# azmyrajab/polars_ols

Hardware: AMD Instinct MI355X
Metric: group_regressions_per_sec (higher is better)
Workload: dtype f32

## Files before the change

### polars_ols_amd/csrc/k4x_inverse.hip

```cpp
#include "k4_rolling.hpp"

namespace pols {

constexpr int KX_MAX = 128;

template <typename T>
struct XCtx {
    const K4Args &a;
    int64_t s;
    int first_chunk;
    int K, LD, NS, tid;
    double *P, *xs, *v, *bv, *beta, *red;
    const T *mycol;
    __device__ XCtx(const K4Args &a_, int64_t s_, int fc, double *lds) : a(a_), s(s_), first_chunk(fc) {
        K = a.k; LD = K | 1; NS = K * K + K; tid = threadIdx.x;
        P = lds; xs = P + (size_t)K * LD; v = xs + KX_MAX + 2; bv = v + KX_MAX; beta = bv + KX_MAX; red = beta + KX_MAX;
        mycol = tid < K ? static_cast<const T *>(a.xtab ? a.xtab[tid] : a.x[tid]) : static_cast<const T *>(a.y);
    }
    static __host__ __device__ size_t lds_doubles(int K) { return (size_t)K * (K | 1) + 4 * KX_MAX + 2 + 16; }

    __device__ __forceinline__ bool valid(int64_t i) const { return a.valid ? a.valid[s + i] != 0 : true; }
    __device__ __forceinline__ int64_t cnt(int64_t i) const { return a.cnt ? (int64_t)a.cnt[s + i] : i + 1; }
    __device__ __forceinline__ int64_t vidx(int64_t r) const { return a.vidx ? (int64_t)a.vidx[s + r] : r; }

    __device__ __forceinline__ void load_row(int64_t i) const {
        __syncthreads();
        if (tid <= K) xs[tid] = (double)mycol[s + i];
        __syncthreads();
    }
    __device__ double block_sum(double x) const {
        const double w = wave_sum_row3(x);
        __syncthreads();
        if ((tid & 63) == 63) red[tid >> 6] = w;
        __syncthreads();
        return red[0] + red[1] + red[2] + red[3];
    }
    __device__ void zero() const {
        for (int q = tid; q < K * LD; q += 256) P[q] = 0.0;
        if (tid < K) bv[tid] = 0.0;
        __syncthreads();
    }
    __device__ void gram_axpy(const double *src, double sign) const {
        for (int q = tid; q < K * K; q += 256) { const int i = q / K, c = q - i * K; P[i * LD + c] += sign * src[q]; }
        if (tid < K) bv[tid] += sign * src[K * K + tid];
        __syncthreads();
    }
    __device__ void gram_add_row(int64_t i, double sign) const {
        load_row(i);
        for (int q = tid; q < K * K; q += 256) { const int r = q / K, c = q - r * K; P[r * LD + c] += sign * (xs[r] * xs[c]); }
        if (tid < K) bv[tid] += sign * (xs[tid] * xs[K]);
        __syncthreads();
    }
    __device__ void gram_prefix(int64_t i, double sign, int nacc) const {
        if (i < 0) return;
        const int64_t c = i / a.chunk_len;
        gram_axpy(a.totals + (size_t)(first_chunk + c) * nacc, sign);
        for (int64_t j = c * a.chunk_len; j <= i; ++j)
            if (valid(j)) gram_add_row(j, sign);
    }
    __device__ void invert(double alpha) const {
        if (tid < K) P[tid * LD + tid] += alpha;
        __syncthreads();
        for (int j = 0; j < K; ++j) {
            const double p = 1.0 / P[j * LD + j];
            if (tid < K) v[tid] = P[tid * LD + j];
            __syncthreads();
            for (int q = tid; q < K * K; q += 256) {
                const int i = q / K, c = q - i * K;
                double val;
                if (i == j && c == j) val = -p;
                else if (i == j) val = v[c] * p;
                else if (c == j) val = v[i] * p;
                else val = P[i * LD + c] - v[i] * v[c] * p;
                P[i * LD + c] = val;
            }
            __syncthreads();
        }
        for (int q = tid; q < K * K; q += 256) { const int i = q / K, c = q - i * K; P[i * LD + c] = -P[i * LD + c]; }
        __syncthreads();
    }
    __device__ void matvec(const double *x, double *out) const {
        if (tid < K) {
            double acc = 0.0;
            const double *row = P + tid * LD;
            for (int c = 0; c < K; ++c) acc += row[c] * x[c];
            out[tid] = acc;
        }
        __syncthreads();
    }
    __device__ void rank1(double coef) const {
        for (int q = tid; q < K * K; q += 256) { const int i = q / K, c = q - i * K; P[i * LD + c] += coef * (v[i] * v[c]); }
        __syncthreads();
    }
    __device__ void sm_update(double sign) const {
        matvec(xs, v);
        const double xv = block_sum(tid < K ? xs[tid] * v[tid] : 0.0);
        rank1(-sign / (1.0 + sign * xv));
        if (tid < K) bv[tid] += sign * (xs[tid] * xs[K]);
        __syncthreads();
    }
    __device__ void solve_beta() const { matvec(bv, beta); }
    __device__ void store(int64_t i, bool have, T *coef, T *pred) const {
        const int64_t row = s + i;
        const double qnan = __longlong_as_double(0x7ff8000000000000LL);
        if (coef && tid < K) coef[row * K + tid] = (T)(have ? beta[tid] : qnan);
        if (pred) {
            load_row(i);
            const double p = block_sum(tid < K ? xs[tid] * (have ? beta[tid] : qnan) : 0.0);
            if (tid == 0) pred[row] = (T)p;
        }
    }
};

template <typename T, bool RLS>
__global__ void __launch_bounds__(256) kx_totals_kernel(const K4Args a) {
    extern __shared__ double lds[];
    const int64_t c = blockIdx.x;
    const K4Chunk ch = a.chunks[c];
    const K4Group G = a.groups[ch.group];
    XCtx<T> cx(a, G.start, G.first_chunk, lds);
    const int K = cx.K, nacc = cx.NS + (RLS ? 1 : 0);
    cx.zero();
    double decay = 1.0;
    for (int64_t i = ch.t0 - G.start; i < ch.t1 - G.start; ++i)
        if (cx.valid(i)) {
            if (RLS) {
                for (int q = cx.tid; q < K * cx.LD; q += 256) cx.P[q] *= a.ff;
                if (cx.tid < K) cx.bv[cx.tid] *= a.ff;
                decay *= a.ff;
                __syncthreads();
            }
            cx.gram_add_row(i, 1.0);
        }
    double *out = a.totals + (size_t)c * nacc;
    for (int q = cx.tid; q < K * K; q += 256) { const int i = q / K, cc = q - i * K; out[q] = cx.P[i * cx.LD + cc]; }
    if (cx.tid < K) out[K * K + cx.tid] = cx.bv[cx.tid];
    if (RLS && cx.tid == 0) out[cx.NS] = decay;
}

template <typename T>
__global__ void __launch_bounds__(256) kx_rolling_walk_kernel(const K4Args a) {
    extern __shared__ double lds[];
    const int64_t c = blockIdx.x;
    const K4Chunk ch = a.chunks[c];
    const K4Group G = a.groups[ch.group];
    XCtx<T> cx(a, G.start, G.first_chunk, lds);
    const int K = cx.K, nacc = cx.NS;
    const int64_t rel0 = ch.t0 - G.start, rel1 = ch.t1 - G.start;
    const int64_t w = a.window, mpv = G.mpv;
    const bool drop = a.drop_mode != 0;
    T *coef = static_cast<T *>(a.coef);
    T *pred = static_cast<T *>(a.pred);
    const double qnan = __longlong_as_double(0x7ff8000000000000LL);

    if (G.all_nan) {
        for (int64_t i = rel0; i < rel1; ++i) {
            if (coef && cx.tid < K) coef[(G.start + i) * K + cx.tid] = (T)qnan;
            if (pred && cx.tid == 0) pred[G.start + i] = (T)qnan;
        }
        return;
    }
    const int64_t j_min = drop ? 0 : max(mpv - w, (int64_t)0);
    const int64_t c0 = drop ? cx.cnt(mpv - 1) : 0;
    const bool longwarm = drop && c0 > w;
    auto old_of = [&](int64_t i) -> int64_t {
        if (!drop) return i - w;
        const int64_t R = cx.cnt(i) - 1;
        const int64_t r = (longwarm && R - c0 < w) ? R - c0 : R - w;
        return r < 0 ? -1 : cx.vidx(r);
    };
    auto gate = [&](int64_t i) -> bool {
        const int64_t i_start = i >= w ? i - w : 0;
        return cx.cnt(i) - cx.cnt(i_start) >= G.gate_n;
    };
    auto gram_state_at = [&](int64_t i) {
        cx.zero();
        cx.gram_prefix(i, 1.0, nacc);
        const int64_t o = (i >= 0) ? old_of(i) : -1;
        if (o >= j_min && i >= mpv) {
            cx.gram_prefix(o, -1.0, nacc);
            cx.gram_prefix(j_min - 1, 1.0, nacc);
        }
        if (longwarm && i >= mpv && cx.cnt(i) - 1 - c0 >= w) {
            cx.gram_prefix(cx.vidx(c0 - 1), 1.0, nacc);
            cx.gram_prefix(cx.vidx(w - 1), -1.0, nacc);
        }
    };

    bool inverted = false, have = false;
    int64_t prev_old = (rel0 > 0 && rel0 - 1 >= mpv) ? old_of(rel0 - 1) : -1;
    if (rel0 >= mpv && rel0 > 0) {
        int64_t ip = rel0 - 1;
        if (!(drop || ip == mpv - 1 || gate(ip))) {
            for (ip = rel0 - 2; ip >= mpv - 1; --ip)
                if (ip == mpv - 1 || gate(ip)) break;
        }
        gram_state_at(ip);
        cx.invert(a.alpha);
        cx.solve_beta();
        have = true;
        if (ip != rel0 - 1) {
            gram_state_at(rel0 - 1);
            cx.invert(a.alpha);
        }
        inverted = true;
    } else {
        gram_state_at(rel0 - 1);
    }
    for (int64_t i = rel0; i < rel1; ++i) {
        const bool vld = cx.valid(i);
        if (vld) {
            if (inverted) { cx.load_row(i); cx.sm_update(1.0); }
            else cx.gram_add_row(i, 1.0);
        }
        if (i >= mpv && (vld || !drop)) {
            const int64_t no = old_of(i);
            bool sub = false;
            if (drop) sub = (no != prev_old && no >= 0);
            else sub = (no >= j_min && no >= 0 && cx.valid(no));
            if (sub) { cx.load_row(no); cx.sm_update(-1.0); }
            prev_old = no;
        }
        if (i >= mpv - 1) {
            const bool do_solve = (i == mpv - 1) || (drop ? vld : gate(i));
            if (do_solve) {
                if (!inverted) { cx.invert(a.alpha); inverted = true; }
                cx.solve_beta();
                have = true;
            }
        }
        cx.store(i, have, coef, pred);
    }
}

template <typename T>
__global__ void __launch_bounds__(256) kx_rls_walk_kernel(const K4Args a) {
    extern __shared__ double lds[];
    const int64_t c = blockIdx.x;
    const K4Chunk ch = a.chunks[c];
    const K4Group G = a.groups[ch.group];
    XCtx<T> cx(a, G.start, G.first_chunk, lds);
    const int K = cx.K, nacc = cx.NS + 1;
    const int64_t rel0 = ch.t0 - G.start, rel1 = ch.t1 - G.start;
    T *coef = static_cast<T *>(a.coef);
    T *pred = static_cast<T *>(a.pred);
    cx.zero();
    cx.gram_axpy(a.totals + (size_t)c * nacc, 1.0);
    cx.invert(0.0);
    cx.solve_beta();
    const double ff = a.ff;
    for (int64_t i = rel0; i < rel1; ++i) {
        if (cx.valid(i)) {
            cx.load_row(i);
            cx.matvec(cx.xs, cx.v);
            const double xv = cx.block_sum(cx.tid < K ? cx.xs[cx.tid] * cx.v[cx.tid] : 0.0);
            const double xb = cx.block_sum(cx.tid < K ? cx.xs[cx.tid] * cx.beta[cx.tid] : 0.0);
            const double r = 1.0 + xv / ff;
            const double err = cx.xs[K] - xb;
            if (cx.tid < K) cx.beta[cx.tid] += cx.v[cx.tid] / (r * ff) * err;
            const double coef_vv = -1.0 / (r * ff);
            for (int q = cx.tid; q < K * K; q += 256) {
                const int ii = q / K, cc = q - ii * K;
                cx.P[ii * cx.LD + cc] = (cx.P[ii * cx.LD + cc] + coef_vv * (cx.v[ii] * cx.v[cc])) / ff;
            }
            __syncthreads();
        }
        cx.store(i, true, coef, pred);
    }
}

template <typename T>
static int kx_launch_t(pols_ctx *ctx, const K4Args &a, bool rls) {
    const size_t lds = sizeof(double) * XCtx<T>::lds_doubles(a.k);
    const int ns = a.k * a.k + a.k;
    static OncePerDevice attr_once;
    if (attr_once.needed(ctx->device)) {
        const void *fns[4] = {reinterpret_cast<const void *>(&kx_totals_kernel<T, false>), reinterpret_cast<const void *>(&kx_totals_kernel<T, true>),
                              reinterpret_cast<const void *>(&kx_rolling_walk_kernel<T>), reinterpret_cast<const void *>(&kx_rls_walk_kernel<T>)};
        for (const void *f : fns) POLS_HIP(hipFuncSetAttribute(f, hipFuncAttributeMaxDynamicSharedMemorySize, 144 * 1024));
        attr_once.done(ctx->device);
    }
    timing_begin(ctx);
    if (rls) {
        hipLaunchKernelGGL((kx_totals_kernel<T, true>), dim3((unsigned)a.n_chunks), dim3(256), lds, ctx->stream, a);
        chunk_scan_launch(ctx, a, ns, 2);
        hipLaunchKernelGGL((kx_rls_walk_kernel<T>), dim3((unsigned)a.n_chunks), dim3(256), lds, ctx->stream, a);
    } else {
        hipLaunchKernelGGL((kx_totals_kernel<T, false>), dim3((unsigned)a.n_chunks), dim3(256), lds, ctx->stream, a);
        chunk_scan_launch(ctx, a, ns, 0);
        hipLaunchKernelGGL((kx_rolling_walk_kernel<T>), dim3((unsigned)a.n_chunks), dim3(256), lds, ctx->stream, a);
    }
    timing_end(ctx);
    POLS_HIP(hipGetLastError());
    return POLS_OK;
}

int k4x_launch(pols_ctx *ctx, int dtype, const K4Args &a) {
    if (a.k > KX_MAX) return fail(POLS_ERR_UNSUPPORTED, "rolling: %d features > %d", a.k, KX_MAX);
    ctx->last_kernel = dtype == POLS_F32 ? "k4x_rolling_inverse_f32" : "k4x_rolling_inverse_f64";
    return dtype == POLS_F32 ? kx_launch_t<float>(ctx, a, false) : kx_launch_t<double>(ctx, a, false);
}

int k3x_launch(pols_ctx *ctx, int dtype, const K4Args &a) {
    if (a.k > KX_MAX) return fail(POLS_ERR_UNSUPPORTED, "rls: %d features > %d", a.k, KX_MAX);
    ctx->last_kernel = dtype == POLS_F32 ? "k3x_rls_inverse_f32" : "k3x_rls_inverse_f64";
    return dtype == POLS_F32 ? kx_launch_t<float>(ctx, a, true) : kx_launch_t<double>(ctx, a, true);
}

}
```

Measured before the change: 132.6 million.

## Keep inverse matrix in registers and stage row batches through LDS

Moves the K×K inverse and Gram state out of LDS into per-thread registers, with each thread owning a row segment. Input rows are staged into LDS in batches of 64, and the per-row flags and old-row indices are precomputed, so per-row global loads and extra barriers go away. Reductions use DPP and double-buffered scratch to cut synchronisations per update, and kernels are templated on a padded width of 64 or 128. The cost is higher register pressure, more complex code, and larger LDS staging buffers, which may limit occupancy.

```diff
diff --git a/polars_ols_amd/csrc/k4x_inverse.hip b/polars_ols_amd/csrc/k4x_inverse.hip
--- a/polars_ols_amd/csrc/k4x_inverse.hip
+++ b/polars_ols_amd/csrc/k4x_inverse.hip
@@ -1,150 +1,263 @@
 #include "k4_rolling.hpp"
 
+#pragma clang fp contract(off)
+
 namespace pols {
 
 constexpr int KX_MAX = 128;
-
-template <typename T>
+constexpr int KX_SB = 64;
+
+template <int KP>
+struct XGeo {
+    static_assert(KP == 64 || KP == 128, "padded width");
+    static constexpr int NSEG = 256 / KP;
+    static constexpr int CPL = KP / NSEG;
+    static constexpr int VL = KP + 2 * NSEG;
+    static constexpr int YS = VL;
+    static constexpr int XS = VL + 2;
+    static constexpr int HEAD = 5 * VL + 16 + KX_SB + KX_SB / 2 + KP + 2;
+    static __host__ __device__ constexpr int pos(int c) { return c + 2 * (c / CPL); }
+    static constexpr size_t lds_bytes(bool with_out) { return sizeof(double) * (size_t)(HEAD + (with_out ? 2 : 1) * KX_SB * XS); }
+};
+
+__device__ __forceinline__ int64_t kx_uniform(int64_t v) {
+    const int lo = __builtin_amdgcn_readfirstlane((int)(v & 0xffffffffLL));
+    const int hi = __builtin_amdgcn_readfirstlane((int)(v >> 32));
+    return ((int64_t)hi << 32) | (unsigned int)lo;
+}
+
+constexpr int KX_F_VALID = 1, KX_F_GATE = 2, KX_F_OUT_VALID = 4;
+
+template <typename T, int KP>
 struct XCtx {
+    using Geo = XGeo<KP>;
+    static constexpr int NSEG = Geo::NSEG, CPL = Geo::CPL, VL = Geo::VL, YS = Geo::YS, XS = Geo::XS;
     const K4Args &a;
     int64_t s;
     int first_chunk;
-    int K, LD, NS, tid;
-    double *P, *xs, *v, *bv, *beta, *red;
-    const T *mycol;
+    int K, NS, tid, r, seg, c0, c0p, rp, tp;
+    int vt = 0, rt = 0, bt = 0;
+    double *vec, *bv, *beta, *red, *xin, *xout;
+    long long *m_no;
+    int *m_fl;
+    const T **colp;
+    double P[CPL];
+
     __device__ XCtx(const K4Args &a_, int64_t s_, int fc, double *lds) : a(a_), s(s_), first_chunk(fc) {
-        K = a.k; LD = K | 1; NS = K * K + K; tid = threadIdx.x;
-        P = lds; xs = P + (size_t)K * LD; v = xs + KX_MAX + 2; bv = v + KX_MAX; beta = bv + KX_MAX; red = beta + KX_MAX;
-        mycol = tid < K ? static_cast<const T *>(a.xtab ? a.xtab[tid] : a.x[tid]) : static_cast<const T *>(a.y);
-    }
-    static __host__ __device__ size_t lds_doubles(int K) { return (size_t)K * (K | 1) + 4 * KX_MAX + 2 + 16; }
+        K = a.k; NS = K * K + K; tid = threadIdx.x;
+        r = tid / NSEG; seg = tid % NSEG; c0 = seg * CPL; c0p = Geo::pos(c0); rp = Geo::pos(r); tp = Geo::pos(tid < KP ? tid : 0);
+        vec = lds; bv = vec + 2 * VL; beta = bv + VL; red = beta + 2 * VL;
+        m_no = reinterpret_cast<long long *>(red + 16);
+        m_fl = reinterpret_cast<int *>(m_no + KX_SB);
+        colp = reinterpret_cast<const T **>(m_no + KX_SB + KX_SB / 2);
+        xin = lds + Geo::HEAD; xout = xin + KX_SB * XS;
+    }
+    __device__ __forceinline__ void init(bool with_out) {
+        for (int j = tid; j <= K; j += 256)
+            colp[j] = j < K ? static_cast<const T *>(a.xtab ? a.xtab[j] : a.x[j]) : static_cast<const T *>(a.y);
+        const int n = (with_out ? 2 : 1) * KX_SB * XS;
+        for (int q = tid; q < n; q += 256) xin[q] = 0.0;
+        for (int q = tid; q < 5 * VL; q += 256) vec[q] = 0.0;
+        __syncthreads();
+    }
 
     __device__ __forceinline__ bool valid(int64_t i) const { return a.valid ? a.valid[s + i] != 0 : true; }
     __device__ __forceinline__ int64_t cnt(int64_t i) const { return a.cnt ? (int64_t)a.cnt[s + i] : i + 1; }
-    __device__ __forceinline__ int64_t vidx(int64_t r) const { return a.vidx ? (int64_t)a.vidx[s + r] : r; }
-
-    __device__ __forceinline__ void load_row(int64_t i) const {
-        __syncthreads();
-        if (tid <= K) xs[tid] = (double)mycol[s + i];
-        __syncthreads();
-    }
-    __device__ double block_sum(double x) const {
+    __device__ __forceinline__ int64_t vidx(int64_t rr) const { return a.vidx ? (int64_t)a.vidx[s + rr] : rr; }
+
+    __device__ __forceinline__ void stage_cols(double *dst, int64_t ri) const {
+        const int w = __builtin_amdgcn_readfirstlane(tid >> 6);
+        double *row = dst + (tid & 63) * XS;
+        if (ri >= 0) {
+#pragma unroll 8
+            for (int j = w; j <= K; j += 4) row[j < K ? Geo::pos(j) : YS] = (double)colp[j][s + ri];
+        }
+    }
+    __device__ __forceinline__ void stage(int64_t i0, int n) const {
+        __syncthreads();
+        const int q = tid & 63;
+        stage_cols(xin, q < n ? i0 + q : -1);
+        if (tid < n) m_fl[tid] = valid(i0 + tid) ? KX_F_VALID : 0;
+        __syncthreads();
+    }
+    __device__ __forceinline__ const double *row_in(int q) const { return xin + q * XS; }
+    __device__ __forceinline__ const double *row_out(int q) const { return xout + q * XS; }
+    __device__ __forceinline__ int flags(int q) const { return __builtin_amdgcn_readfirstlane(m_fl[q]); }
+
+    __device__ __forceinline__ double block_sum(double x) {
         const double w = wave_sum_row3(x);
-        __syncthreads();
-        if ((tid & 63) == 63) red[tid >> 6] = w;
-        __syncthreads();
-        return red[0] + red[1] + red[2] + red[3];
-    }
-    __device__ void zero() const {
-        for (int q = tid; q < K * LD; q += 256) P[q] = 0.0;
-        if (tid < K) bv[tid] = 0.0;
-        __syncthreads();
-    }
-    __device__ void gram_axpy(const double *src, double sign) const {
-        for (int q = tid; q < K * K; q += 256) { const int i = q / K, c = q - i * K; P[i * LD + c] += sign * src[q]; }
-        if (tid < K) bv[tid] += sign * src[K * K + tid];
-        __syncthreads();
-    }
-    __device__ void gram_add_row(int64_t i, double sign) const {
-        load_row(i);
-        for (int q = tid; q < K * K; q += 256) { const int r = q / K, c = q - r * K; P[r * LD + c] += sign * (xs[r] * xs[c]); }
-        if (tid < K) bv[tid] += sign * (xs[tid] * xs[K]);
-        __syncthreads();
-    }
-    __device__ void gram_prefix(int64_t i, double sign, int nacc) const {
+        double *rd = red + 8 * rt; rt ^= 1;
+        if ((tid & 63) == 63) rd[tid >> 6] = w;
+        __syncthreads();
+        return (rd[0] + rd[1]) + (rd[2] + rd[3]);
+    }
+    template <typename F>
+    __device__ __forceinline__ void for_piece(const double *v, F &&f) const {
+        constexpr int BL = CPL > 16 ? 16 : CPL, NB = CPL / BL;
+        double blk[2][BL];
+        auto load = [&](int b) __attribute__((always_inline)) {
+#pragma unroll
+            for (int q = 0; q < BL; q += 2) {
+                const double2 t = *reinterpret_cast<const double2 *>(v + c0p + b * BL + q);
+                blk[b & 1][q] = t.x; blk[b & 1][q + 1] = t.y;
+            }
+        };
+        load(0);
+#pragma unroll
+        for (int b = 0; b < NB; ++b) {
+            if (b + 1 < NB) load(b + 1);
+            __builtin_amdgcn_sched_barrier(0);
+#pragma unroll
+            for (int q = 0; q < BL; ++q) f(b * BL + q, blk[b & 1][q]);
+            __builtin_amdgcn_sched_barrier(0);
+        }
+    }
+    __device__ __forceinline__ double row_dot(const double *x) const {
+        double acc[4] = {0.0, 0.0, 0.0, 0.0};
+        for_piece(x, [&](int cc, double xc) __attribute__((always_inline)) { acc[cc & 3] = fma(P[cc], xc, acc[cc & 3]); });
+        double v = (acc[0] + acc[1]) + (acc[2] + acc[3]);
+        asm volatile("" : "+v"(v));
+        v += dpp_get<0xB1>(v);
+        if constexpr (NSEG == 4) v += dpp_get<0x4E>(v);
+        return v;
+    }
+    __device__ __forceinline__ void rank1(const double *v, double coef) {
+        const double vr = v[rp];
+        for_piece(v, [&](int cc, double vc) __attribute__((always_inline)) { P[cc] = fma(coef, vr * vc, P[cc]); });
+    }
+
+    __device__ __forceinline__ void zero() {
+        __syncthreads();
+#pragma unroll
+        for (int cc = 0; cc < CPL; ++cc) P[cc] = 0.0;
+        if (tid < VL) bv[tid] = 0.0;
+        __syncthreads();
+    }
+    __device__ __forceinline__ void gram_axpy(const double *src, double sign) {
+        if (r < K) {
+            const double *row = src + (size_t)r * K + c0;
+#pragma unroll
+            for (int cc = 0; cc < CPL; ++cc)
+                if (c0 + cc < K) P[cc] += sign * row[cc];
+        }
+        if (tid < K) bv[tp] += sign * src[K * K + tid];
+    }
+    __device__ __forceinline__ void gram_add_row(const double *row, double sign) {
+        const double xr = row[rp];
+        for_piece(row, [&](int cc, double xc) __attribute__((always_inline)) { P[cc] += sign * (xr * xc); });
+        if (tid < K) bv[tp] += sign * (row[tp] * row[YS]);
+    }
+    __device__ __forceinline__ void gram_prefix(int64_t i, double sign, int nacc) {
         if (i < 0) return;
         const int64_t c = i / a.chunk_len;
         gram_axpy(a.totals + (size_t)(first_chunk + c) * nacc, sign);
-        for (int64_t j = c * a.chunk_len; j <= i; ++j)
-            if (valid(j)) gram_add_row(j, sign);
-    }
-    __device__ void invert(double alpha) const {
-        if (tid < K) P[tid * LD + tid] += alpha;
-        __syncthreads();
+        for (int64_t j0 = c * a.chunk_len; j0 <= i; j0 += KX_SB) {
+            const int n = (int)min((int64_t)KX_SB, i - j0 + 1);
+            stage(j0, n);
+            for (int q = 0; q < n; ++q)
+                if (flags(q) & KX_F_VALID) gram_add_row(row_in(q), sign);
+        }
+    }
+    __device__ __forceinline__ void invert(double alpha) {
+#pragma unroll
+        for (int cc = 0; cc < CPL; ++cc)
+            if (c0 + cc == r && r < K) P[cc] += alpha;
         for (int j = 0; j < K; ++j) {
-            const double p = 1.0 / P[j * LD + j];
-            if (tid < K) v[tid] = P[tid * LD + j];
+            double *cb = vec + VL * vt; vt ^= 1;
+            if (r == j) {
+#pragma unroll
+                for (int cc = 0; cc < CPL; cc += 2) *reinterpret_cast<double2 *>(cb + c0p + cc) = make_double2(P[cc], P[cc + 1]);
+            }
             __syncthreads();
-            for (int q = tid; q < K * K; q += 256) {
-                const int i = q / K, c = q - i * K;
-                double val;
-                if (i == j && c == j) val = -p;
-                else if (i == j) val = v[c] * p;
-                else if (c == j) val = v[i] * p;
-                else val = P[i * LD + c] - v[i] * v[c] * p;
-                P[i * LD + c] = val;
-            }
-            __syncthreads();
-        }
-        for (int q = tid; q < K * K; q += 256) { const int i = q / K, c = q - i * K; P[i * LD + c] = -P[i * LD + c]; }
-        __syncthreads();
-    }
-    __device__ void matvec(const double *x, double *out) const {
-        if (tid < K) {
-            double acc = 0.0;
-            const double *row = P + tid * LD;
-            for (int c = 0; c < K; ++c) acc += row[c] * x[c];
-            out[tid] = acc;
-        }
-        __syncthreads();
-    }
-    __device__ void rank1(double coef) const {
-        for (int q = tid; q < K * K; q += 256) { const int i = q / K, c = q - i * K; P[i * LD + c] += coef * (v[i] * v[c]); }
-        __syncthreads();
-    }
-    __device__ void sm_update(double sign) const {
-        matvec(xs, v);
-        const double xv = block_sum(tid < K ? xs[tid] * v[tid] : 0.0);
-        rank1(-sign / (1.0 + sign * xv));
-        if (tid < K) bv[tid] += sign * (xs[tid] * xs[K]);
-        __syncthreads();
-    }
-    __device__ void solve_beta() const { matvec(bv, beta); }
-    __device__ void store(int64_t i, bool have, T *coef, T *pred) const {
+            const double p = 1.0 / cb[Geo::pos(j)];
+            const bool prow = r == j;
+            if (prow) {
+#pragma unroll
+                for (int cc = 0; cc < CPL; ++cc) P[cc] = 0.0;
+            }
+            const double vr = prow ? -1.0 : cb[rp];
+            const double colv = prow ? -p : vr * p;
+            const int jc = j - c0;
+            for_piece(cb, [&](int cc, double vc) __attribute__((always_inline)) { P[cc] = cc == jc ? colv : fma(-(vr * vc), p, P[cc]); });
+        }
+#pragma unroll
+        for (int cc = 0; cc < CPL; ++cc) P[cc] = -P[cc];
+    }
+    __device__ __forceinline__ void sm_update(const double *row, double sign) {
+        const double xr = row[rp];
+        const double pv = row_dot(row);
+        const double w = wave_sum_row3(seg == 0 ? xr * pv : 0.0);
+        double *vb = vec + VL * vt; vt ^= 1;
+        double *rd = red + 8 * rt; rt ^= 1;
+        if (seg == 0) vb[rp] = pv;
+        if ((tid & 63) == 63) rd[tid >> 6] = w;
+        if (tid < K) bv[tp] += sign * (row[tp] * row[YS]);
+        __syncthreads();
+        const double xv = (rd[0] + rd[1]) + (rd[2] + rd[3]);
+        rank1(vb, -sign / (1.0 + sign * xv));
+    }
+    __device__ __forceinline__ void solve_beta() {
+        const double pv = row_dot(bv);
+        bt ^= 1;
+        if (seg == 0) beta[VL * bt + rp] = pv;
+        __syncthreads();
+    }
+    __device__ __forceinline__ void store(int64_t i, const double *xrow, bool have, T *coef, T *pred) {
         const int64_t row = s + i;
         const double qnan = __longlong_as_double(0x7ff8000000000000LL);
-        if (coef && tid < K) coef[row * K + tid] = (T)(have ? beta[tid] : qnan);
+        const double b = (have && tid < K) ? beta[VL * bt + tp] : qnan;
+        if (coef && tid < K) coef[row * K + tid] = (T)b;
         if (pred) {
-            load_row(i);
-            const double p = block_sum(tid < K ? xs[tid] * (have ? beta[tid] : qnan) : 0.0);
+            const double p = block_sum(tid < K ? xrow[tp] * b : 0.0);
             if (tid == 0) pred[row] = (T)p;
         }
     }
 };
 
-template <typename T, bool RLS>
+template <typename T, int KP, bool RLS>
 __global__ void __launch_bounds__(256) kx_totals_kernel(const K4Args a) {
-    extern __shared__ double lds[];
+    extern __shared__ __align__(16) double lds[];
     const int64_t c = blockIdx.x;
     const K4Chunk ch = a.chunks[c];
     const K4Group G = a.groups[ch.group];
-    XCtx<T> cx(a, G.start, G.first_chunk, lds);
-    const int K = cx.K, nacc = cx.NS + (RLS ? 1 : 0);
+    XCtx<T, KP> cx(a, G.start, G.first_chunk, lds);
+    constexpr int CPL = XCtx<T, KP>::CPL;
+    const int K = cx.K;
+    cx.init(false);
     cx.zero();
     double decay = 1.0;
-    for (int64_t i = ch.t0 - G.start; i < ch.t1 - G.start; ++i)
-        if (cx.valid(i)) {
-            if (RLS) {
-                for (int q = cx.tid; q < K * cx.LD; q += 256) cx.P[q] *= a.ff;
-                if (cx.tid < K) cx.bv[cx.tid] *= a.ff;
-                decay *= a.ff;
-                __syncthreads();
-            }
-            cx.gram_add_row(i, 1.0);
-        }
-    double *out = a.totals + (size_t)c * nacc;
-    for (int q = cx.tid; q < K * K; q += 256) { const int i = q / K, cc = q - i * K; out[q] = cx.P[i * cx.LD + cc]; }
-    if (cx.tid < K) out[K * K + cx.tid] = cx.bv[cx.tid];
+    const int64_t rel1 = ch.t1 - G.start;
+    for (int64_t i0 = ch.t0 - G.start; i0 < rel1; i0 += KX_SB) {
+        const int n = (int)min((int64_t)KX_SB, rel1 - i0);
+        cx.stage(i0, n);
+        for (int q = 0; q < n; ++q)
+            if (cx.flags(q) & KX_F_VALID) {
+                if (RLS) {
+#pragma unroll
+                    for (int cc = 0; cc < CPL; ++cc) cx.P[cc] *= a.ff;
+                    if (cx.tid < K) cx.bv[cx.tp] *= a.ff;
+                    decay *= a.ff;
+                }
+                cx.gram_add_row(cx.row_in(q), 1.0);
+            }
+    }
+    double *out = a.totals + (size_t)c * (cx.NS + (RLS ? 1 : 0));
+    if (cx.r < K) {
+#pragma unroll
+        for (int cc = 0; cc < CPL; ++cc)
+            if (cx.c0 + cc < K) out[(size_t)cx.r * K + cx.c0 + cc] = cx.P[cc];
+    }
+    if (cx.tid < K) out[K * K + cx.tid] = cx.bv[cx.tp];
     if (RLS && cx.tid == 0) out[cx.NS] = decay;
 }
 
-template <typename T>
+template <typename T, int KP>
 __global__ void __launch_bounds__(256) kx_rolling_walk_kernel(const K4Args a) {
-    extern __shared__ double lds[];
+    extern __shared__ __align__(16) double lds[];
     const int64_t c = blockIdx.x;
     const K4Chunk ch = a.chunks[c];
     const K4Group G = a.groups[ch.group];
-    XCtx<T> cx(a, G.start, G.first_chunk, lds);
+    XCtx<T, KP> cx(a, G.start, G.first_chunk, lds);
     const int K = cx.K, nacc = cx.NS;
     const int64_t rel0 = ch.t0 - G.start, rel1 = ch.t1 - G.start;
     const int64_t w = a.window, mpv = G.mpv;
@@ -160,151 +273,191 @@
         }
         return;
     }
+    cx.init(true);
     const int64_t j_min = drop ? 0 : max(mpv - w, (int64_t)0);
     const int64_t c0 = drop ? cx.cnt(mpv - 1) : 0;
     const bool longwarm = drop && c0 > w;
-    auto old_of = [&](int64_t i) -> int64_t {
+    auto old_of = [&](int64_t i) __attribute__((always_inline)) -> int64_t {
         if (!drop) return i - w;
         const int64_t R = cx.cnt(i) - 1;
         const int64_t r = (longwarm && R - c0 < w) ? R - c0 : R - w;
         return r < 0 ? -1 : cx.vidx(r);
     };
-    auto gate = [&](int64_t i) -> bool {
+    auto gate = [&](int64_t i) __attribute__((always_inline)) -> bool {
         const int64_t i_start = i >= w ? i - w : 0;
         return cx.cnt(i) - cx.cnt(i_start) >= G.gate_n;
     };
-    auto gram_state_at = [&](int64_t i) {
+    auto gram_state_at = [&](int64_t i) __attribute__((always_inline)) {
         cx.zero();
-        cx.gram_prefix(i, 1.0, nacc);
         const int64_t o = (i >= 0) ? old_of(i) : -1;
-        if (o >= j_min && i >= mpv) {
-            cx.gram_prefix(o, -1.0, nacc);
-            cx.gram_prefix(j_min - 1, 1.0, nacc);
-        }
-        if (longwarm && i >= mpv && cx.cnt(i) - 1 - c0 >= w) {
-            cx.gram_prefix(cx.vidx(c0 - 1), 1.0, nacc);
-            cx.gram_prefix(cx.vidx(w - 1), -1.0, nacc);
-        }
+        const bool slid = o >= j_min && i >= mpv;
+        const bool kept = longwarm && i >= mpv && cx.cnt(i) - 1 - c0 >= w;
+        for (int t = 0; t < 5; ++t) {
+            int64_t at = -1;
+            double sign = 1.0;
+            if (t == 0) at = i;
+            else if (t == 1) { if (slid) { at = o; sign = -1.0; } }
+            else if (t == 2) { if (slid) at = j_min - 1; }
+            else if (t == 3) { if (kept) at = cx.vidx(c0 - 1); }
+            else if (kept) { at = cx.vidx(w - 1); sign = -1.0; }
+            cx.gram_prefix(at, sign, nacc);
+        }
+    };
+    auto stage_walk = [&](int64_t i0, int n) __attribute__((always_inline)) {
+        __syncthreads();
+        const int q = cx.tid & 63;
+        const int64_t i = i0 + q;
+        int64_t no = -1;
+        int fl = 0;
+        if (q < n) {
+            if (cx.valid(i)) fl |= KX_F_VALID;
+            if (i >= mpv) no = old_of(i);
+            if (!drop && i >= mpv - 1 && gate(i)) fl |= KX_F_GATE;
+            if (no >= 0 && cx.valid(no)) fl |= KX_F_OUT_VALID;
+        }
+        cx.stage_cols(cx.xin, q < n ? i : -1);
+        cx.stage_cols(cx.xout, no);
+        if (cx.tid < n) { cx.m_fl[cx.tid] = fl; cx.m_no[cx.tid] = no; }
+        __syncthreads();
     };
 
     bool inverted = false, have = false;
     int64_t prev_old = (rel0 > 0 && rel0 - 1 >= mpv) ? old_of(rel0 - 1) : -1;
-    if (rel0 >= mpv && rel0 > 0) {
-        int64_t ip = rel0 - 1;
-        if (!(drop || ip == mpv - 1 || gate(ip))) {
-            for (ip = rel0 - 2; ip >= mpv - 1; --ip)
-                if (ip == mpv - 1 || gate(ip)) break;
-        }
-        gram_state_at(ip);
-        cx.invert(a.alpha);
-        cx.solve_beta();
-        have = true;
-        if (ip != rel0 - 1) {
-            gram_state_at(rel0 - 1);
+    const bool carry = rel0 >= mpv && rel0 > 0;
+    int64_t ip = rel0 - 1;
+    if (carry && !(drop || ip == mpv - 1 || gate(ip))) {
+        for (ip = rel0 - 2; ip >= mpv - 1; --ip)
+            if (ip == mpv - 1 || gate(ip)) break;
+    }
+    const int n_pass = (carry && ip != rel0 - 1) ? 2 : 1;
+    for (int pass = 0; pass < n_pass; ++pass) {
+        gram_state_at(pass == n_pass - 1 ? rel0 - 1 : ip);
+        if (carry) {
             cx.invert(a.alpha);
-        }
-        inverted = true;
-    } else {
-        gram_state_at(rel0 - 1);
+            if (pass == 0) { cx.solve_beta(); have = true; }
+            inverted = true;
+        }
     }
     for (int64_t i = rel0; i < rel1; ++i) {
-        const bool vld = cx.valid(i);
+        const int q = (int)((i - rel0) % KX_SB);
+        if (q == 0) stage_walk(i, (int)min((int64_t)KX_SB, rel1 - i));
+        const int fl = cx.flags(q);
+        const bool vld = (fl & KX_F_VALID) != 0;
         if (vld) {
-            if (inverted) { cx.load_row(i); cx.sm_update(1.0); }
-            else cx.gram_add_row(i, 1.0);
+            if (inverted) cx.sm_update(cx.row_in(q), 1.0);
+            else cx.gram_add_row(cx.row_in(q), 1.0);
         }
         if (i >= mpv && (vld || !drop)) {
-            const int64_t no = old_of(i);
+            const int64_t no = kx_uniform(cx.m_no[q]);
             bool sub = false;
             if (drop) sub = (no != prev_old && no >= 0);
-            else sub = (no >= j_min && no >= 0 && cx.valid(no));
-            if (sub) { cx.load_row(no); cx.sm_update(-1.0); }
+            else sub = (no >= j_min && no >= 0 && (fl & KX_F_OUT_VALID) != 0);
+            if (sub) cx.sm_update(cx.row_out(q), -1.0);
             prev_old = no;
         }
         if (i >= mpv - 1) {
-            const bool do_solve = (i == mpv - 1) || (drop ? vld : gate(i));
+            const bool do_solve = (i == mpv - 1) || (drop ? vld : (fl & KX_F_GATE) != 0);
             if (do_solve) {
                 if (!inverted) { cx.invert(a.alpha); inverted = true; }
                 cx.solve_beta();
                 have = true;
             }
         }
-        cx.store(i, have, coef, pred);
-    }
-}
-
-template <typename T>
+        cx.store(i, cx.row_in(q), have, coef, pred);
+    }
+}
+
+template <typename T, int KP>
 __global__ void __launch_bounds__(256) kx_rls_walk_kernel(const K4Args a) {
-    extern __shared__ double lds[];
+    extern __shared__ __align__(16) double lds[];
     const int64_t c = blockIdx.x;
     const K4Chunk ch = a.chunks[c];
     const K4Group G = a.groups[ch.group];
-    XCtx<T> cx(a, G.start, G.first_chunk, lds);
+    XCtx<T, KP> cx(a, G.start, G.first_chunk, lds);
+    using Cx = XCtx<T, KP>;
+    constexpr int VL = Cx::VL;
     const int K = cx.K, nacc = cx.NS + 1;
     const int64_t rel0 = ch.t0 - G.start, rel1 = ch.t1 - G.start;
     T *coef = static_cast<T *>(a.coef);
     T *pred = static_cast<T *>(a.pred);
+    cx.init(false);
     cx.zero();
     cx.gram_axpy(a.totals + (size_t)c * nacc, 1.0);
     cx.invert(0.0);
     cx.solve_beta();
-    const double ff = a.ff;
-    for (int64_t i = rel0; i < rel1; ++i) {
-        if (cx.valid(i)) {
-            cx.load_row(i);
-            cx.matvec(cx.xs, cx.v);
-            const double xv = cx.block_sum(cx.tid < K ? cx.xs[cx.tid] * cx.v[cx.tid] : 0.0);
-            const double xb = cx.block_sum(cx.tid < K ? cx.xs[cx.tid] * cx.beta[cx.tid] : 0.0);
-            const double r = 1.0 + xv / ff;
-            const double err = cx.xs[K] - xb;
-            if (cx.tid < K) cx.beta[cx.tid] += cx.v[cx.tid] / (r * ff) * err;
-            const double coef_vv = -1.0 / (r * ff);
-            for (int q = cx.tid; q < K * K; q += 256) {
-                const int ii = q / K, cc = q - ii * K;
-                cx.P[ii * cx.LD + cc] = (cx.P[ii * cx.LD + cc] + coef_vv * (cx.v[ii] * cx.v[cc])) / ff;
-            }
-            __syncthreads();
-        }
-        cx.store(i, true, coef, pred);
-    }
-}
-
-template <typename T>
+    const double ff = a.ff, rff = 1.0 / ff;
+    double *bb = cx.beta + VL * cx.bt;
+    for (int64_t i0 = rel0; i0 < rel1; i0 += KX_SB) {
+        const int n = (int)min((int64_t)KX_SB, rel1 - i0);
+        cx.stage(i0, n);
+        for (int q = 0; q < n; ++q) {
+            const double *row = cx.row_in(q);
+            if (cx.flags(q) & KX_F_VALID) {
+                const double xr = row[cx.rp];
+                const double pv = cx.row_dot(row);
+                const double w1 = wave_sum_row3(cx.seg == 0 ? xr * pv : 0.0);
+                const double w2 = wave_sum_row3(cx.tid < K ? row[cx.tp] * bb[cx.tp] : 0.0);
+                double *vb = cx.vec + VL * cx.vt; cx.vt ^= 1;
+                double *rd = cx.red + 8 * cx.rt; cx.rt ^= 1;
+                if (cx.seg == 0) vb[cx.rp] = pv;
+                if ((cx.tid & 63) == 63) { rd[cx.tid >> 6] = w1; rd[4 + (cx.tid >> 6)] = w2; }
+                __syncthreads();
+                const double xv = (rd[0] + rd[1]) + (rd[2] + rd[3]);
+                const double xb = (rd[4] + rd[5]) + (rd[6] + rd[7]);
+                const double r = 1.0 + xv / ff;
+                const double err = row[Cx::YS] - xb;
+                if (cx.tid < K) bb[cx.tp] += vb[cx.tp] / (r * ff) * err;
+                const double coef_vv = -1.0 / (r * ff);
+                const double vr = vb[cx.rp];
+                cx.for_piece(vb, [&](int cc, double vc) __attribute__((always_inline)) { cx.P[cc] = fma(coef_vv, vr * vc, cx.P[cc]) * rff; });
+            }
+            cx.store(i0 + q, row, true, coef, pred);
+        }
+    }
+}
+
+template <typename T, int KP>
 static int kx_launch_t(pols_ctx *ctx, const K4Args &a, bool rls) {
-    const size_t lds = sizeof(double) * XCtx<T>::lds_doubles(a.k);
-    const int ns = a.k * a.k + a.k;
+    using Geo = XGeo<KP>;
+    static_assert(Geo::lds_bytes(true) <= 160 * 1024, "LDS of one CU");
     static OncePerDevice attr_once;
     if (attr_once.needed(ctx->device)) {
-        const void *fns[4] = {reinterpret_cast<const void *>(&kx_totals_kernel<T, false>), reinterpret_cast<const void *>(&kx_totals_kernel<T, true>),
-                              reinterpret_cast<const void *>(&kx_rolling_walk_kernel<T>), reinterpret_cast<const void *>(&kx_rls_walk_kernel<T>)};
-        for (const void *f : fns) POLS_HIP(hipFuncSetAttribute(f, hipFuncAttributeMaxDynamicSharedMemorySize, 144 * 1024));
+        const void *fns[4] = {reinterpret_cast<const void *>(&kx_totals_kernel<T, KP, false>), reinterpret_cast<const void *>(&kx_totals_kernel<T, KP, true>),
+                              reinterpret_cast<const void *>(&kx_rolling_walk_kernel<T, KP>), reinterpret_cast<const void *>(&kx_rls_walk_kernel<T, KP>)};
+        for (const void *f : fns) POLS_HIP(hipFuncSetAttribute(f, hipFuncAttributeMaxDynamicSharedMemorySize, (int)Geo::lds_bytes(true)));
         attr_once.done(ctx->device);
     }
+    const int ns = a.k * a.k + a.k;
     timing_begin(ctx);
     if (rls) {
-        hipLaunchKernelGGL((kx_totals_kernel<T, true>), dim3((unsigned)a.n_chunks), dim3(256), lds, ctx->stream, a);
+        hipLaunchKernelGGL((kx_totals_kernel<T, KP, true>), dim3((unsigned)a.n_chunks), dim3(256), Geo::lds_bytes(false), ctx->stream, a);
         chunk_scan_launch(ctx, a, ns, 2);
-        hipLaunchKernelGGL((kx_rls_walk_kernel<T>), dim3((unsigned)a.n_chunks), dim3(256), lds, ctx->stream, a);
+        hipLaunchKernelGGL((kx_rls_walk_kernel<T, KP>), dim3((unsigned)a.n_chunks), dim3(256), Geo::lds_bytes(false), ctx->stream, a);
     } else {
-        hipLaunchKernelGGL((kx_totals_kernel<T, false>), dim3((unsigned)a.n_chunks), dim3(256), lds, ctx->stream, a);
+        hipLaunchKernelGGL((kx_totals_kernel<T, KP, false>), dim3((unsigned)a.n_chunks), dim3(256), Geo::lds_bytes(false), ctx->stream, a);
         chunk_scan_launch(ctx, a, ns, 0);
-        hipLaunchKernelGGL((kx_rolling_walk_kernel<T>), dim3((unsigned)a.n_chunks), dim3(256), lds, ctx->stream, a);
+        hipLaunchKernelGGL((kx_rolling_walk_kernel<T, KP>), dim3((unsigned)a.n_chunks), dim3(256), Geo::lds_bytes(true), ctx->stream, a);
     }
     timing_end(ctx);
     POLS_HIP(hipGetLastError());
     return POLS_OK;
 }
 
+template <typename T>
+static int kx_launch_w(pols_ctx *ctx, const K4Args &a, bool rls) {
+    return a.k <= 64 ? kx_launch_t<T, 64>(ctx, a, rls) : kx_launch_t<T, 128>(ctx, a, rls);
+}
+
 int k4x_launch(pols_ctx *ctx, int dtype, const K4Args &a) {
     if (a.k > KX_MAX) return fail(POLS_ERR_UNSUPPORTED, "rolling: %d features > %d", a.k, KX_MAX);
     ctx->last_kernel = dtype == POLS_F32 ? "k4x_rolling_inverse_f32" : "k4x_rolling_inverse_f64";
-    return dtype == POLS_F32 ? kx_launch_t<float>(ctx, a, false) : kx_launch_t<double>(ctx, a, false);
+    return dtype == POLS_F32 ? kx_launch_w<float>(ctx, a, false) : kx_launch_w<double>(ctx, a, false);
 }
 
 int k3x_launch(pols_ctx *ctx, int dtype, const K4Args &a) {
     if (a.k > KX_MAX) return fail(POLS_ERR_UNSUPPORTED, "rls: %d features > %d", a.k, KX_MAX);
     ctx->last_kernel = dtype == POLS_F32 ? "k3x_rls_inverse_f32" : "k3x_rls_inverse_f64";
-    return dtype == POLS_F32 ? kx_launch_t<float>(ctx, a, true) : kx_launch_t<double>(ctx, a, true);
-}
-
-}
+    return dtype == POLS_F32 ? kx_launch_w<float>(ctx, a, true) : kx_launch_w<double>(ctx, a, true);
+}
+
+}
```

Result: no change. 132.9 million (median of 6 runs) (+0.2%).
